# OxygenLost/dddmr_navigation

Measured on AMD Instinct MI355X. Metric: scored trajectories/sec (N_traj x N_steps), higher is better.
Workload: dtype f32; 1 GPU; C3: 16384 trajectories x 80 steps vs 500000-point cloud, 80-pose prune plan, shipped critic stack; scene_layout=r02, trajectories_per_gpu=16384, steps_per_trajectory=80, parallelism=single, contexts_per_gpu=1

## Files before the change

dddmr_navigation_amd/_capi.py:

```python
from __future__ import annotations

import ctypes as C
import os

MAX_CRITICS = 8
NAME_LEN = 64
ABI_VERSION = 2

OK = 0
ERR_BAD_ARG = -1
ERR_NO_DEVICE = -2
ERR_HIP = -3
ERR_UNKNOWN_THEORY = -4
ERR_CAPACITY = -5
ERR_STATE = -6
OPINION_PASS = 0
OPINION_PATH_BLOCKED_WAIT = 1

TF_FAIL = 0
PRUNE_PLAN_FAIL = 1
ALL_TRAJECTORIES_FAIL = 2
PERCEPTION_MALFUNCTION = 3
TRAJECTORY_FOUND = 4
PATH_BLOCKED_WAIT = 5
# ... 291 lines not shown
_get = (_int, [_ctx, _vp, _sz, _pn])
_get_of = (_int, [_ctx, _i32, _vp, _sz, _pn])
_fixed = (_int, [_ctx, _vp, _sz])
_plain = (_int, [_ctx])

_TABLE = {
    "create": (_int, [_P(RolloutConfig), _P(_ctx)]),
    "destroy": (None, [_ctx]),
    "set_cloud": (_int, [_ctx] + _cloud),
    "set_scan": (_int, [_ctx] + _cloud + [_pd, _pd, _dbl, _dbl, _pu]),
    "set_stitcher": (_int, [_ctx, _i32]),
    "get_cloud": _get,
    "set_prune_plan": _fixed,
    "samples": (_int, [_ctx, _str, _P(TickInput), _vp, _sz, _pn]),
    "tick": (_int, [_ctx, _str, _P(TickInput), _P(RolloutResult)]),
    "tick_begin": (_int, [_ctx, _str, _P(TickInput)]),
    "tick_end": (_int, [_ctx, _P(RolloutResult)]),
    "resolve": (_int, [_ctx, _i64, _P(RolloutResult)]),
    "winner_words": (None, [_P(RolloutResult), _pi64]),
    "resolve_words": (_int, [_ctx, _pi64, _i32, _P(RolloutResult)]),
    "get_debug": (_int, [_ctx, _P(RolloutDebug)]),
    "heading_rows": _plain,
    "fused_walk": _plain,
    "get_best_poses": _get,
    "get_best_cuboids": _get,
    "get_pose_arrays": _get_of,
    "path_blocked": (_int, [_ctx, _vp, _sz, _dbl, _pd, _P(_i32), _vp]),
    "pack_key": (_i64, [_dbl, _u32]),
    "key_index": (_i32, [_i64]),
    "comm_unique_id": (_int, [_vp]),
    "comm_init": (_int, [_ctx, _vp, _i32, _i32]),
    "comm_destroy": _plain,
    "comm_ranks": (_int, [_ctx, _P(_i32)]),
    "device_count": (_int, [_P(_i32)]),
    "comm_loopback": _plain,
    "comm_loopback_set_peer": (_int, [_ctx, _i32, _pi64]),
    "marking_create": (_int, [_ctx, _P(MarkingConfig)] + _cloud + _cloud),
    "marking_update": (_int, [_ctx, _pd, _pd, _P(MarkingStats)]),
    "marking_reset": _plain,
    "marking_get_voxels": _get,
    "marking_get_points": (_int, [_ctx, _vp, _vp, _sz, _pn]),
    "marking_get_dgraph": _fixed,
    "marking_get_lethal": _fixed,
    "marking_route_counts": (_int, [_ctx, _pu, _pu, _pu]),
    "set_scan_source": (_int, [_ctx, _i32] + _cloud + [_pd, _pd, _dbl, _dbl, _pu, _pu]),
    "set_stitcher_source": (_int, [_ctx, _i32, _i32]),
# ... 86 lines not shown
```

dddmr_navigation_amd/csrc/rollout_engine.hip:

```cpp
#include <hip/hip_runtime.h>
#include <dlfcn.h>
#include <rccl/rccl.h>

#include <algorithm>
#include <atomic>
#include <cmath>
#include <cstdarg>
#include <chrono>
#include <cstdio>
#include <cstdlib>
#include <cstring>
#include <memory>
#include <mutex>
#include <string>
#include <vector>

#include "rollout_kernels.hip.h"
#include "tick_plan.hip.h"
#include "perception_kernels.hip.h"
#include "depth_feed.hip.h"
#include "depth_image.hip.h"
#include "depth_clear.hip.h"
#include "lidar_sweep.hip.h"
#include "lidar_features.hip.h"
// ... 96 lines not shown
  bool comm_loopback = false;
  int64_t* slots_dev = nullptr;
  int64_t* slots_red = nullptr;
  DevResult* local_result_dev = nullptr;

  ModuleSlot<MarkingState> marking;
  ModuleSlot<DepthMarkState> dmark;
  ModuleSlot<DepthLayerState> dlayer;
  ModuleSlot<StackState> stack;
  ModuleSlot<MclState> mcl;

  std::mutex tick_mu;
  std::mutex err_mu;
  std::string last_error;

  DevTick last{};
  bool have_last = false;
  Window last_window;
  int timing = 1;
  int timing_every = 1;
  int spin = 1;
  int last_heading_rows = -1;
  int last_fused_walk = -1;
  uint32_t seq = 0;
  DevResult last_result{};
  float last_score_ms = 0.f, last_device_ms = 0.f;
  struct Pending {
    bool active = false;
    TickPlan plan;
    bool timed = false, timed_all = false;
    Window window;
  } pend;
};

namespace {

class CloudPin {
 public:
  enum Mode { kFront, kOfPendingTick, kAdopted };
  explicit CloudPin(dddmr_rollout_ctx* c, Mode mode = kFront) : c_(c), owns_(mode != kOfPendingTick) {
    if (mode == kAdopted) {
      idx_ = c_->busy;
      return;
    }
    std::lock_guard<std::mutex> lk(c_->cloud_mu);
    if (mode == kFront) {
// ... 64 lines not shown
}
#define TICK_IDLE(ctx, what)                        \
  std::lock_guard<std::mutex> tk((ctx)->tick_mu);   \
  if ((ctx)->pend.active) return refuse_pending(ctx, what)

const dddmr_theory_config* find_theory(const dddmr_rollout_ctx* ctx, const char* name) {
  for (const auto& t : ctx->theories)
    if (std::strncmp(t.name, name, DDDMR_NAME_LEN) == 0) return &t;
  return nullptr;
}

void read_env(dddmr_rollout_ctx* ctx) {
  TickKnobs& kn = ctx->knobs;
  if (const char* e = std::getenv("DDDMR_CELL")) {
    const float v = (float)std::atof(e);
    if (v > 0.01f && v < 10.f) { kn.cell_size = v; kn.cell_forced = true; }
  }
  if (const char* e = std::getenv("DDDMR_TILE")) kn.tile_override = std::atoi(e);
  if (const char* e = std::getenv("DDDMR_RT")) kn.rt_override = std::atoi(e);
  if (const char* e = std::getenv("DDDMR_THREADS")) kn.threads_override = std::atoi(e) == 512 ? 512 : 256;
  if (const char* e = std::getenv("DDDMR_TAIL_ROUND")) kn.tail_round = std::atoi(e) != 0;
  if (const char* e = std::getenv("DDDMR_HEADING_ROWS")) kn.heading_rows = std::atoi(e) != 0;
  if (const char* e = std::getenv("DDDMR_FUSE_WALK")) kn.fuse_walk = std::atoi(e) != 0;
  if (const char* e = std::getenv("DDDMR_FINAL")) kn.final_mode = std::atoi(e) ? 1 : 0;
  if (const char* e = std::getenv("DDDMR_PROBE")) kn.probe_mode = std::atoi(e) ? 1 : 0;
  if (const char* e = std::getenv("DDDMR_TIMING")) ctx->timing = std::atoi(e);
  if (const char* e = std::getenv("DDDMR_TIMING_EVERY")) ctx->timing_every = std::max(1, std::atoi(e));
  if (const char* e = std::getenv("DDDMR_SPIN")) ctx->spin = std::atoi(e);
  const struct { const char* name; bool* on; } given[] = {
      {"DDDMR_NO_ASSIGN", &kn.no_assign}, {"DDDMR_NO_BOXFAST", &kn.no_boxfast}, {"DDDMR_NO_TAB", &kn.no_tab},
      {"DDDMR_GNZ_ONE", &kn.gnz_one},     {"DDDMR_POISON", &ctx->poison},       {"DDDMR_HOST_PROF", &ctx->host_prof},
      {"DDDMR_DEBUG_GRID", &ctx->debug_grid}};
  for (const auto& g : given) *g.on = std::getenv(g.name) != nullptr;
  if (const char* e = std::getenv("DDDMR_CEIL_BLOCKS")) ctx->ceil_blocks = std::max(1, std::atoi(e));
}

}

#include "rollout_comm.hip.h"

extern "C" {

const char* dddmr_rollout_version(void) { return "dddmr-rollout-mi355x 0.1 (gfx950)"; }

size_t dddmr_rollout_sizeof(int which) {
  switch (which) {
// ... 123 lines not shown
    HIPCHK(ctx, dev_alloc(mem, &ctx->steps, N));
    HIPCHK(ctx, dev_alloc(mem, &ctx->samples_out, N));
    HIPCHK(ctx, dev_alloc(mem, &ctx->best_key, (size_t)kSlotBase + (size_t)kSlotWords * N));
    HIPCHK(ctx, dev_alloc(mem, &ctx->overflow, 1));
    HIPCHK(ctx, dev_alloc(mem, &ctx->traj_load, N));
    HIPCHK(ctx, hipMemset(ctx->traj_load, 0, N * sizeof(uint32_t)));
    HIPCHK(ctx, dev_alloc(mem, &ctx->assign, N));
    HIPCHK(ctx, dev_alloc(mem, &ctx->tickets, 2));
    HIPCHK(ctx, hipMemset(ctx->tickets, 0, 2 * sizeof(uint32_t)));
    HIPCHK(ctx, dev_alloc(mem, &ctx->poses_dev, (size_t)cfg->max_steps * 7));
    HIPCHK(ctx, dev_alloc(mem, &ctx->blocked_plan, (size_t)kBlockedMaxPlan));
    HIPCHK(ctx, dev_alloc(mem, &ctx->blocked_flags, (size_t)kBlockedMaxPlan / 32));
    for (int i = 0; i < kCloudBufs; ++i) HIPCHK(ctx, host_alloc(ctx->host, &ctx->cloud_stage[i], P * sizeof(float4)));
    const size_t small = std::max<size_t>({3 * kMaxAxis * sizeof(float), N * sizeof(float4),
                                           plan_cap * sizeof(float4)});
    HIPCHK(ctx, host_alloc(ctx->host, &ctx->small_stage, small));
    if (host_mapped_alloc(ctx->host, &ctx->result_host, &ctx->result_dev, sizeof(DevResult)) != 0)
      return fail(ctx, DDDMR_ERR_HIP, "result record allocation failed");
    const int rc = perception_alloc(ctx->feed, P);
    if (rc != 0) return fail(ctx, DDDMR_ERR_HIP, "perception scratch allocation failed");
    {
      const void* big_lds_kernels[] = {
          reinterpret_cast<const void*>(k_rollout), reinterpret_cast<const void*>(k_bin_count),
          reinterpret_cast<const void*>(k_score<256, false, false>), reinterpret_cast<const void*>(k_score<256, false, true>),
          reinterpret_cast<const void*>(k_score<256, true, false>),  reinterpret_cast<const void*>(k_score<256, true, true>),
          reinterpret_cast<const void*>(k_score<512, false, false>), reinterpret_cast<const void*>(k_score<512, false, true>),
          reinterpret_cast<const void*>(k_score<512, true, false>),  reinterpret_cast<const void*>(k_score<512, true, true>)};
      for (const void* f : big_lds_kernels) HIPCHK(ctx, hipFuncSetAttribute(f, hipFuncAttributeMaxDynamicSharedMemorySize, kScoreLdsMax));
    }
    HIPCHK(ctx, hipDeviceSynchronize());
    return DDDMR_OK;
  };
  const int rc = init();
  if (rc != DDDMR_OK) {
    fprintf(stderr, "dddmr_rollout_create: %s\n", ctx->last_error.c_str());
    dddmr_rollout_destroy(ctx);
    return rc;
  }
  *out = ctx;
  return DDDMR_OK;
}

static void publish_cloud(dddmr_rollout_ctx* ctx, int idx, uint32_t n, const SourceLayout& layout) {
  std::lock_guard<std::mutex> lk(ctx->cloud_mu);
  ctx->cloud_n[idx] = n;
  ctx->cloud_layout[idx] = layout;
  ctx->front = idx;
  ctx->wait_pending[idx] = true;
}

// ... 198 lines not shown
      ctx->st_cap = cap;
      if (!ctx->traj_info) HIPCHK(ctx, dev_alloc(ctx->mem, &ctx->traj_info, (size_t)ctx->cfg.max_trajectories));
    }
  }
  HIPCHK(ctx, pin.wait_on(ctx->stream));

  const auto prof_t1 = std::chrono::steady_clock::now();
  if (ctx->poison && k.n_local > 0) {
    HIPCHK(ctx, hipMemsetAsync(ctx->costs, 0xFF, (size_t)k.n_local * sizeof(double), ctx->stream));
    HIPCHK(ctx, hipMemsetAsync(ctx->steps, 0xFF, (size_t)k.n_local * sizeof(int32_t), ctx->stream));
    HIPCHK(ctx, hipMemsetAsync(ctx->samples_out, 0xFF, (size_t)k.n_local * sizeof(float4), ctx->stream));
    HIPCHK(ctx, hipMemsetAsync(ctx->partial, 0xFF, (size_t)k.n_local * sizeof(TrajPartial), ctx->stream));
    HIPCHK(ctx, hipMemsetAsync(ctx->st_pp, 0xFF, (size_t)k.n_local * sizeof(double2), ctx->stream));
  }
  k.seq = ++ctx->seq;
  if (k.seq == 0) k.seq = ctx->seq = 1;
  const bool timed = ctx->timing >= 1 && (ctx->seq % (uint32_t)ctx->timing_every) == 0;
  const bool timed_all = timed && ctx->timing >= 2;
  if (timed_all) HIPCHK(ctx, hipEventRecord(ctx->ev0, ctx->stream));
  ctx->feedback.load_theory = theory_id;
  ctx->feedback.load_nlocal = k.n_local;
  ctx->last_heading_rows = p.heading_rows;
  ctx->last_fused_walk = k.n_local > 0 ? p.fused_walk : 0;
  drain.armed = true;
  if (k.n_points > 0) {
    hipLaunchKernelGGL(k_bin_count, dim3(p.cnt_blocks + p.roll_blocks + (k.use_assign ? k.assign_groups : 0)), dim3(kBinThreads),
                       p.roll_launch_lds, ctx->stream, k, pin.dev(), ctx->cell_count, ctx->cell_start, ctx->pt_slot, ctx->tickets,
                       ctx->best_key, ctx->overflow, ctx->axes_dev, ctx->samples_dev, ctx->traj_info, ctx->st_sc,
                       ctx->st_xy, ctx->st_pp, ctx->traj_load, ctx->assign, p.heading_rows);
    hipLaunchKernelGGL(k_bin_scatter, dim3(p.bin_blocks), dim3(256), 0, ctx->stream, k, pin.dev(),
                       ctx->pt_slot, ctx->cell_start, ctx->sorted, ctx->row_tab);
  } else {
    hipLaunchKernelGGL(k_bin_reset, dim3(1), dim3(256), 0, ctx->stream, k, ctx->cell_count, ctx->cell_start,
                       ctx->best_key, ctx->overflow);
    if (p.roll_blocks > 0)
      hipLaunchKernelGGL(k_rollout, dim3(p.roll_blocks), dim3(256), p.roll_launch_lds, ctx->stream, k, ctx->axes_dev,
                         ctx->samples_dev, ctx->traj_info, ctx->st_sc, ctx->st_xy, ctx->st_pp, p.heading_rows);
    if (k.use_assign)
      hipLaunchKernelGGL(k_assign, dim3(k.assign_groups), dim3(kBinThreads), 0, ctx->stream, k, ctx->traj_load, ctx->assign);
  }
  if (timed) HIPCHK(ctx, hipEventRecord(ctx->evs0, ctx->stream));
  DevResult* score_result = exchange ? ctx->local_result_dev : ctx->result_dev;
  int64_t* score_words = exchange ? ctx->slots_dev + 2 * p.rank : nullptr;
  if (k.n_local > 0) {
    const int wgs = k.n_tiles;
    const size_t lds = p.score_lds;
#define DDDMR_LAUNCH_SCORE(T, L)                                                                                   \
  do { if (k.probe) DDDMR_LAUNCH_SCORE_P(T, L, true); else DDDMR_LAUNCH_SCORE_P(T, L, false); } while (0)
#define DDDMR_LAUNCH_SCORE_P(T, L, P)                                                                              \
  hipLaunchKernelGGL((k_score<T, L, P>), dim3(wgs), dim3(T), lds, ctx->stream, k, ctx->traj_info, ctx->st_sc,     \
                     ctx->st_xy, ctx->plan_dev, ctx->cell_start, ctx->sorted, ctx->costs, ctx->steps,             \
                     ctx->samples_out, ctx->best_key, ctx->overflow, ctx->tickets + 1, score_result, ctx->assign, \
                     ctx->traj_load, score_words, ctx->row_tab, ctx->plan_pairs_dev, ctx->partial, p.fused_walk,  \
                     ctx->st_pp)
    if (p.thr == 512) { if (p.lean) DDDMR_LAUNCH_SCORE(512, true); else DDDMR_LAUNCH_SCORE(512, false); }
    else              { if (p.lean) DDDMR_LAUNCH_SCORE(256, true); else DDDMR_LAUNCH_SCORE(256, false); }
#undef DDDMR_LAUNCH_SCORE
#undef DDDMR_LAUNCH_SCORE_P
  } else {
    hipLaunchKernelGGL(k_empty_result, dim3(1), dim3(64), 0, ctx->stream, k, ctx->cell_start, score_result, score_words);
  }
  if (timed) HIPCHK(ctx, hipEventRecord(ctx->evs1, ctx->stream));
  if (k.n_local > 0 && k.final_kernel)
    hipLaunchKernelGGL(k_finalize, dim3((k.n_local + kFinalThreads - 1) / kFinalThreads), dim3(kFinalThreads), 0, ctx->stream, k,
                       ctx->traj_info, ctx->partial, ctx->costs, ctx->steps, ctx->samples_out, ctx->traj_load, ctx->best_key,
                       ctx->cell_start, ctx->overflow, ctx->tickets + 1, score_result, score_words);
  if (exchange) {
    if (ctx->comm) {
      const int nrc = rccl().all_reduce(ctx->slots_dev, ctx->slots_red, (size_t)2 * ctx->comm_ranks, ncclInt64, ncclMin,
                                        ctx->comm, ctx->stream);
      if (nrc != ncclSuccess) return fail(ctx, DDDMR_ERR_HIP, "ncclAllReduce failed: %s", rccl().error_string((ncclResult_t)nrc));
    } else {
      HIPCHK(ctx, hipMemcpyAsync(ctx->slots_red, ctx->slots_dev, (size_t)2 * ctx->comm_ranks * sizeof(int64_t),
                                 hipMemcpyDeviceToDevice, ctx->stream));
    }
    hipLaunchKernelGGL(k_resolve, dim3(1), dim3(64), 0, ctx->stream, k, ctx->slots_red, ctx->comm_ranks,
                       ctx->local_result_dev, ctx->axes_dev, ctx->samples_dev, ctx->result_dev);
  }
  if (timed_all) HIPCHK(ctx, hipEventRecord(ctx->ev1, ctx->stream));
  HIPCHK(ctx, hipGetLastError());
  if (ctx->host_prof) {
// ... 159 lines not shown
  if (!th) return fail(ctx, DDDMR_ERR_UNKNOWN_THEORY, "unknown theory '%s'", theory_name);
  Window w;
  make_window(*th, *in, w);
  const size_t n = w.count();
  *n_samples = n;
  if (!samples_out) return DDDMR_OK;
  if (capacity < n) return fail(ctx, DDDMR_ERR_CAPACITY, "samples: capacity %zu < %zu", capacity, n);
  for (size_t i = 0; i < n; ++i) sample_of(w, (int)i, samples_out + 3 * i, samples_out + 3 * i + 1, samples_out + 3 * i + 2);
  return DDDMR_OK;
}

int dddmr_rollout_heading_rows(dddmr_rollout_ctx* ctx) {
  if (!ctx) return -1;
  std::lock_guard<std::mutex> tk(ctx->tick_mu);
  return ctx->last_heading_rows;
}

int dddmr_rollout_fused_walk(dddmr_rollout_ctx* ctx) {
  if (!ctx) return -1;
  std::lock_guard<std::mutex> tk(ctx->tick_mu);
  return ctx->last_fused_walk;
}

int dddmr_rollout_get_debug(dddmr_rollout_ctx* ctx, dddmr_rollout_debug* dbg) {
  if (!ctx || !dbg) return DDDMR_ERR_BAD_ARG;
  std::lock_guard<std::mutex> tk(ctx->tick_mu);
  if (!ctx->have_last) return fail(ctx, DDDMR_ERR_STATE, "get_debug before any tick");
  if (ctx->pend.active) return refuse_pending(ctx, "get_debug");
  HIPCHK(ctx, hipSetDevice(ctx->device));
  HIPCHK(ctx, hipStreamSynchronize(ctx->stream));
  const size_t n = (size_t)ctx->last.n_local;
  if (n == 0) return DDDMR_OK;
  if (dbg->costs) HIPCHK(ctx, hipMemcpy(dbg->costs, ctx->costs, n * sizeof(double), hipMemcpyDeviceToHost));
  if (dbg->steps) HIPCHK(ctx, hipMemcpy(dbg->steps, ctx->steps, n * sizeof(int32_t), hipMemcpyDeviceToHost));
  if (dbg->samples) {
    std::vector<float4> tmp(n);
    HIPCHK(ctx, hipMemcpy(tmp.data(), ctx->samples_out, n * sizeof(float4), hipMemcpyDeviceToHost));
    for (size_t i = 0; i < n; ++i) {
      dbg->samples[3 * i + 0] = tmp[i].x;
      dbg->samples[3 * i + 1] = tmp[i].y;
      dbg->samples[3 * i + 2] = tmp[i].z;
    }
  }
  return DDDMR_OK;
}

// ... 104 lines not shown
```

dddmr_navigation_amd/csrc/rollout_kernels.hip.h:

```cpp
#pragma once
#include <hip/hip_runtime.h>
#include <limits.h>
#include <stdint.h>

#include "../../include/dddmr_rollout.h"

#pragma clang fp contract(off)

namespace dddmr {

#ifndef DDDMR_PSPLIT_MAX
#define DDDMR_PSPLIT_MAX 4
#endif
#ifndef DDDMR_SCORE_WPE
#define DDDMR_SCORE_WPE 2
#endif
#ifndef DDDMR_SCORE_WPE_256
#define DDDMR_SCORE_WPE_256 5
#endif
#ifdef DDDMR_HANDOFF_ACQREL
#define DDDMR_HANDOFF_ORDER __ATOMIC_ACQ_REL
#else
#define DDDMR_HANDOFF_ORDER __ATOMIC_RELAXED
#endif
// ... 620 lines not shown
  for (int idx = tid; idx < nt * S1; idx += kThreads) {
    const int j = bj, s = bs;
    bj += stride_j;
    bs += stride_s;
    if (bs >= S1) { bs -= S1; ++bj; }
    if (s < steps_s[j]) {
      const float* slot = reinterpret_cast<const float*>(inc + idx);
      st_xy[(size_t)li_s[j] * k.max_steps + s] = make_float2(slot[0], slot[2]);
    }
  }
  if (tid < nt) {
    const int ns = steps_s[tid];
    double2 pp = make_double2(0.0, 0.0);
    if (ns > 0) {
      const float* slot = reinterpret_cast<const float*>(inc + (size_t)tid * S1 + (ns - 1));
      const double2 cs = shared ? hrow[(int)lc_s[tid] * S1 + ns] : inc[(size_t)tid * S1 + ns];
      pp = pure_pursuit_last_pose(k, make_float2(slot[0], slot[2]), cs);
    }
    st_pp[li_s[tid]] = pp;
  }
  DDDMR_RSTAMP(3);
}

__device__ __forceinline__ int tile_round_base(const DevTick& k, int r) {
  return r < k.r0 ? r * k.nb_tiles : k.r0 * k.nb_tiles + (r - k.r0) * k.n_tiles;
}
__device__ __forceinline__ int tile_slot(const DevTick& k, int b, int j) {
  return tile_round_base(k, b < k.nb_tiles ? j : j + k.r0) + b;
}
constexpr int kAssignPer = 4;
template <int kThreads>
__device__ __forceinline__ void assign_block(const DevTick& k, const int grp, const uint32_t* __restrict__ load,
                                             uint32_t* __restrict__ assign) {
  __shared__ uint32_t hist[kLoadClasses];
  __shared__ uint32_t wsum[kThreads / 64];
  __shared__ uint32_t mx_s, mn_s;
  static_assert(kLoadClasses == kThreads, "one class per lane in the scan");
  const int tid = threadIdx.x;
  const int G = k.assign_groups;
  const int n = k.n_local, tl = k.n_tiles / G, tlb = k.nb_tiles / G;
  const int ng = (n - grp + G - 1) / G;
  auto group_slot = [&](int r) {
    const int early = k.r0 * tlb;
    int start, width, round;
    if (r < early) { round = r / tlb; start = round * tlb; width = tlb; }
    else { round = k.r0 + (r - early) / tl; start = early + (round - k.r0) * tl; width = tl; }
    const int pos = r - start;
    const int bl = ((round & 1) && start + width <= ng) ? width - 1 - pos : pos;
    return grp + G * (start + bl);
  };
  DDDMR_RSTAMP(0);
  hist[tid] = 0;
  if (tid == 0) { mx_s = 1; mn_s = 0xFFFFFFFFu; }
  uint32_t v[kAssignPer];
  uint32_t mx = 1, mn = 0xFFFFFFFFu;
#pragma unroll
  for (int e = 0; e < kAssignPer; ++e) {
    const int m = tid + e * kThreads;
    v[e] = m < ng ? load[grp + G * m] : 0u;
    if (m < ng) { mx = max(mx, v[e]); mn = min(mn, v[e]); }
  }
#pragma unroll
  for (int o = 32; o > 0; o >>= 1) {
    mx = max(mx, (uint32_t)__shfl_xor((int)mx, o, 64));
    mn = min(mn, (uint32_t)__shfl_xor((int)mn, o, 64));
  }
  __syncthreads();
  if ((tid & 63) == 0) { atomicMax(&mx_s, mx); atomicMin(&mn_s, mn); }
  __syncthreads();
  if (mx_s <= mn_s) {
#pragma unroll
    for (int e = 0; e < kAssignPer; ++e) {
      const int m = tid + e * kThreads;
// ... 2 lines not shown
    return;
  }
  const float scale = (float)(kLoadClasses - 1) / (float)mx_s;
#pragma unroll
  for (int e = 0; e < kAssignPer; ++e) {
    const int m = tid + e * kThreads;
    if (m < ng) atomicAdd(&hist[kLoadClasses - 1 - min(kLoadClasses - 1, (int)((float)v[e] * scale))], 1u);
  }
  __syncthreads();
  const uint32_t cnt = hist[tid];
  const uint32_t inc = wave_incl_scan_u32(cnt);
  if ((tid & 63) == 63) wsum[tid >> 6] = inc;
  __syncthreads();
  uint32_t base = inc - cnt;
  for (int w = 0; w < (tid >> 6); ++w) base += wsum[w];
  hist[tid] = base;
  __syncthreads();
#pragma unroll
  for (int e = 0; e < kAssignPer; ++e) {
    const int m = tid + e * kThreads;
    if (m < ng) {
      const int c = kLoadClasses - 1 - min(kLoadClasses - 1, (int)((float)v[e] * scale));
      const int r = (int)atomicAdd(&hist[c], 1u);
      assign[group_slot(r)] = (uint32_t)(grp + G * m);
    }
  }
  DDDMR_RSTAMP(3);
}

__global__ __launch_bounds__(kBinThreads) void k_assign(DevTick k, const uint32_t* __restrict__ load,
                                                        uint32_t* __restrict__ assign) {
  assign_block<kBinThreads>(k, (int)blockIdx.x, load, assign);
}

__global__ __launch_bounds__(256) void k_rollout(DevTick k, const float* __restrict__ axes,
                                                 const float4* __restrict__ samples,
                                                 TrajInfo* __restrict__ info, double2* __restrict__ st_sc,
                                                 float2* __restrict__ st_xy, double2* __restrict__ st_pp,
                                                 const int heading_rows) {
  extern __shared__ __attribute__((aligned(16))) unsigned char dyn_lds[];
  rollout_block<256>(k, (int)blockIdx.x, axes, samples, info, st_sc, st_xy, st_pp, dyn_lds, heading_rows != 0);
}

__global__ __launch_bounds__(kBinThreads, 8) void k_bin_count(DevTick k, const float4* __restrict__ cloud,
                                                   uint32_t* __restrict__ cell_count,
                                                   uint32_t* __restrict__ cell_start,
                                                   uint2* __restrict__ pt_slot, uint32_t* __restrict__ ticket,
                                                   int64_t* __restrict__ best_key,
                                                   uint32_t* __restrict__ overflow, const float* __restrict__ axes,
                                                   const float4* __restrict__ samples, TrajInfo* __restrict__ info,
                                                   double2* __restrict__ st_sc, float2* __restrict__ st_xy,
                                                   double2* __restrict__ st_pp, const uint32_t* __restrict__ load,
                                                   uint32_t* __restrict__ assign, const int heading_rows) {
  extern __shared__ __attribute__((aligned(16))) unsigned char dyn_lds[];
  const int n_assign = k.use_assign ? k.assign_groups : 0;
  if ((int)blockIdx.x < n_assign) {
    assign_block<kBinThreads>(k, (int)blockIdx.x, load, assign);
    return;
  }
  if ((int)blockIdx.x < n_assign + k.roll_blocks) {
    rollout_block<kBinThreads>(k, (int)blockIdx.x - n_assign, axes, samples, info, st_sc, st_xy, st_pp, dyn_lds, heading_rows != 0);
    return;
  }
  const int bin_block = (int)blockIdx.x - n_assign - k.roll_blocks;
  __shared__ uint32_t wave_sum[16];
  __shared__ uint32_t carry_s;
  __shared__ uint32_t is_last;
  const int stride = k.bin_blocks * blockDim.x;
  DDDMR_RSTAMP(0);
  for (int base = bin_block * blockDim.x + threadIdx.x; base < k.n_points; base += stride * kBinPer) {
    float4 p[kBinPer];
    uint2 slot[kBinPer];
#pragma unroll
    for (int m = 0; m < kBinPer; ++m) {
      const int i = base + m * stride;
      p[m] = i < k.n_points ? cloud[i] : make_float4(0.f, 0.f, 0.f, 0.f);
    }
#pragma unroll
    for (int m = 0; m < kBinPer; ++m) {
      const int i = base + m * stride;
// ... 318 lines not shown
    *result = r;
    if (words_out) {
      words_out[0] = any ? (int64_t)bc : kKeyNone;
      words_out[1] = any ? -(int64_t)r.index : kKeyNone;
    } else {
      __threadfence_system();
      __hip_atomic_store(&result->seq, k.seq, __ATOMIC_RELEASE, __HIP_MEMORY_SCOPE_SYSTEM);
    }
    if (kStamps) DDDMR_STAMP_RAW(18);
  }
}

__device__ __forceinline__ double stick_sum_wave(const float* dr, const int ns, const int lane) {
  double acc = 0.0;
  for (int s2 = lane; s2 < ns; s2 += 64) acc += (double)dr[s2];
  acc += dpp_row_shl<8>(acc);
  acc += dpp_row_shl<4>(acc);
  acc += dpp_row_shl<2>(acc);
  acc += dpp_row_shl<1>(acc);
  const double r1 = __shfl(acc, 16, 64), r2 = __shfl(acc, 32, 64), r3 = __shfl(acc, 48, 64);
  return (acc + r1) + (r2 + r3);
}

template <int kScoreThreads, bool kLean, bool kProbe>
__global__ __launch_bounds__(kScoreThreads, kScoreThreads >= 512 ? DDDMR_SCORE_WPE : DDDMR_SCORE_WPE_256) void k_score(
    DevTick k, const TrajInfo* __restrict__ info, const double2* __restrict__ st_sc, const float2* __restrict__ st_xy,
    const float4* __restrict__ plan_xyz, const uint32_t* __restrict__ cell_start,
    const Pt3* __restrict__ sorted, double* __restrict__ costs, int32_t* __restrict__ steps_out,
    float4* __restrict__ samples_out, int64_t* __restrict__ best_key, uint32_t* __restrict__ overflow,
    uint32_t* __restrict__ ticket, DevResult* __restrict__ result, const uint32_t* __restrict__ assign,
    uint32_t* __restrict__ traj_load, int64_t* __restrict__ words_out, const uint32_t* __restrict__ row_tab,
    const float* __restrict__ plan_pairs, TrajPartial* __restrict__ partial, const int fused_walk,
    const double2* __restrict__ st_pp) {
  extern __shared__ __attribute__((aligned(16))) unsigned char lds_raw[];
  const int tile = k.tile;
  const int S1 = k.max_steps + 1;
  const int Qcap = tile * k.max_steps;
  constexpr bool kCanFuse = kLean && kScoreThreads == 512;
  const bool fused = kCanFuse && fused_walk != 0 && Qcap <= kScoreThreads && k.m > 0 && k.want_collision != 0 && k.n_points >= 5;
  const bool need_box = k.want_collision != 0, need_mm = !kLean && k.want_minmax != 0;
  const bool rec_pose = !kLean && k.rec_pose != 0;
  const bool box_fast = kLean || k.box_fast != 0;
  const int rec_words = rec_words_of(rec_pose, need_mm);
  const int mm_ofs = kRecBase + (rec_pose ? 3 : 0);
  size_t ofs = 0;
  TrajHead* head = reinterpret_cast<TrajHead*>(lds_raw);
  ofs += sizeof(TrajHead) * (size_t)tile;
  ofs = (ofs + 15) & ~(size_t)15;
  float4* plan = reinterpret_cast<float4*>(lds_raw + ofs);
  ofs += 16 * (size_t)(k.m > 0 ? k.m : 1);
  float4* ppos = reinterpret_cast<float4*>(lds_raw + ofs);
  ofs += 16 * (size_t)Qcap;
  float* dist = reinterpret_cast<float*>(lds_raw + ofs);
  ofs += 4 * (size_t)tile * S1;
  float* rec = reinterpret_cast<float*>(lds_raw + ofs);
  ofs += 4 * (size_t)rec_words * Qcap;
// ... 481 lines not shown
        const int i1 = min(k.m, i + per);
        for (; i + 4 <= i1; i += 4) {
          const float4 p0 = plan[i], p1 = plan[i + 1], p2 = plan[i + 2], p3 = plan[i + 3];
          const f2 da = l2_simple2(f2{p0.x, p1.x}, f2{p0.y, p1.y}, f2{p0.z, p1.z}, px, py, pz);
          const f2 db = l2_simple2(f2{p2.x, p3.x}, f2{p2.y, p3.y}, f2{p2.z, p3.z}, px, py, pz);
          best = fminf(fminf(best, fminf(da.x, da.y)), fminf(db.x, db.y));
        }
        for (; i < i1; ++i) {
          const float4 pp = plan[i];
          best = fminf(best, l2_simple(pp.x, pp.y, pp.z, px, py, pz));
        }
      }
      if (G > 1) best = fminf(best, dpp_row_shl<1>(best));
      if (G > 2) best = fminf(best, dpp_row_shl<2>(best));
      if (G > 4) best = fminf(best, dpp_row_shl<4>(best));
      if (G > 8) best = fminf(best, dpp_row_shl<8>(best));
      if (valid && g == 0) dist[(size_t)j * S1 + s] = sqrtf(best);
    }
  }
  __syncthreads();
  }
  DDDMR_STAMP(8);

  if (k.final_kernel) {
    for (int j = wid; j < nt; j += kScoreThreads / 64) {
      const int ns = head[j].steps;
      const double sum = stick_sum_wave(dist + (size_t)j * S1, ns, lane);
      if (lane == 0) {
        const bool hb = head[j].hit_box != 0, hm = head[j].hit_mm != 0;
        const bool dead = cloud_ok && ((need_box && hb) || (need_mm && hm));
        TrajPartial* pr = partial + head[j].li;
        pr->stick_sum = dead ? 0.0 : sum;
        pr->pp_dist = head[j].pp_dist;
        pr->pp_yaw = head[j].pp_yaw;
        pr->dist_last = (ns > 0 && !dead) ? dist[(size_t)j * S1 + ns - 1] : 0.f;
        pr->flags = partial_flags(head[j].walked, hb, hm);
      }
    }
    DDDMR_STAMP(10);
    DDDMR_STAMP(11);
    DDDMR_STAMP(7);
    return;
  }
  for (int j = wid; j < nt; j += kScoreThreads / 64) {
    const double sum = stick_sum_wave(dist + (size_t)j * S1, head[j].steps, lane);
    if (lane == 0) head[j].stick_sum = sum;
  }
  __syncthreads();
  DDDMR_STAMP(10);

  int64_t cbits = kKeyNone;
  int my_gi = -1;
  if (tid < nt) {
    const TrajHead h = head[tid];
    const int li = head[tid].li;
    const int gi = k.begin + li;
    my_gi = gi;
    const bool hb = h.hit_box != 0, hm = h.hit_mm != 0;
    const bool dead = cloud_ok && ((need_box && hb) || (need_mm && hm));
    double cost = DDDMR_COST_NOT_GENERATED;
    if (h.steps > 0) {
      const float dist_last = dead ? 0.f : dist[(size_t)tid * S1 + h.steps - 1];
      StackArgs sa;
      stack_args_load(k, sa);
      asm volatile("" : "+s"(sa.kind), "+s"(sa.w), "+s"(sa.tw), "+s"(sa.ow));
      cost = score_stack(k, sa, h.w, h.steps, hb, hm, h.stick_sum, h.pp_dist, h.pp_yaw, dist_last, &cbits);
    }
    costs[li] = cost;
    samples_out[li] = make_float4(h.vx, h.vy, h.w, 0.f);
    steps_out[li] = h.steps;
    traj_load[li] = traj_load_of(k.m, h.walked, h.steps, (need_box && hb) || (need_mm && hm));
  }
  DDDMR_STAMP(11);
  unsigned long long* slots = reinterpret_cast<unsigned long long*>(best_key) + kSlotBase;
  if (tid < 64) {
    long long cc = (long long)cbits;
    int gi_w = my_gi;
    {
      long long oc; int oi; bool take;
      oc = dpp_row_shl<8>(cc); oi = dpp_row_shl<8>(gi_w); take = oc < cc || (oc == cc && oi > gi_w); cc = take ? oc : cc; gi_w = take ? oi : gi_w;
      oc = dpp_row_shl<4>(cc); oi = dpp_row_shl<4>(gi_w); take = oc < cc || (oc == cc && oi > gi_w); cc = take ? oc : cc; gi_w = take ? oi : gi_w;
      oc = dpp_row_shl<2>(cc); oi = dpp_row_shl<2>(gi_w); take = oc < cc || (oc == cc && oi > gi_w); cc = take ? oc : cc; gi_w = take ? oi : gi_w;
      oc = dpp_row_shl<1>(cc); oi = dpp_row_shl<1>(gi_w); take = oc < cc || (oc == cc && oi > gi_w); cc = take ? oc : cc; gi_w = take ? oi : gi_w;
    }
    const int win_gi = __builtin_amdgcn_readfirstlane(gi_w);
    const bool gen = tid < nt && head[tid].steps > 0;
    const bool coll = gen && cloud_ok && ((need_box && head[tid].hit_box) || (need_mm && head[tid].hit_mm));
    const unsigned long long cm = __ballot(coll), gm = __ballot(gen);
    const unsigned long long wm = __ballot(tid < nt && my_gi == win_gi);
    if (tid == 0) {
      float vx = 0.f, vy = 0.f, w = 0.f;
      if (cc != (long long)kKeyNone && wm) {
        const int wl = __ffsll((long long)wm) - 1;
        vx = head[wl].vx; vy = head[wl].vy; w = head[wl].w;
// ... 265 lines not shown
```

dddmr_navigation_amd/csrc/tick_plan.hip.h:

```cpp
#pragma once
#include <algorithm>
#include <cmath>
#include <cstring>
#include <string>
#include <vector>

#include "rollout_kernels.hip.h"

using namespace dddmr;

namespace {

constexpr uint32_t kCapCells = 1u << 20;
constexpr int kMaxAxis = 4096;
constexpr int kScoreLdsMax = 150 * 1024;

struct Window {
  std::vector<float> ax, ay, ath;
  bool list_mode = false;
  std::vector<float4> list;
  size_t count() const { return list_mode ? list.size() : ax.size() * ay.size() * ath.size(); }
};

void velocity_samples(double lo, double hi, int n, bool insert_zero, std::vector<float>& out) {
// ... 166 lines not shown
  } else {
    const int nth = (int)w.ath.size(), ny = (int)w.ay.size();
    *vx = w.ax[(idx / nth) / ny];
    *vy = w.ay[(idx / nth) % ny];
    *wz = w.ath[idx % nth];
  }
}

struct TickKnobs {
  float cell_size = 0.25f;
  bool cell_forced = false;
  bool gnz_one = false;
  int tile_override = 0;
  int threads_override = 0;
  int rt_override = 0;
  bool tail_round = false;
  int final_mode = -1;
  int probe_mode = -1;
  bool no_assign = false;
  bool no_boxfast = false;
  bool no_tab = false;
  bool heading_rows = true;
  bool fuse_walk = true;
  int n_cu = 256;
};

struct TickFeedback {
  int load_theory = -1, load_nlocal = -1;
  float collided_share = 1.0f;
};

enum SampleUpload {
  kUploadNone = 0,
  kUploadList,
  kUploadAxesInline,
  kUploadAxesDev
};

struct TickPlan {
  DevTick k{};
  int s_tick = 0;
  int rank = 0;
  int thr = 512;
  size_t score_lds = 0;
  bool lean = false;
  int cnt_blocks = 0;
  int bin_blocks = 0;
  int roll_blocks = 0;
  size_t roll_lds = 0;
  int heading_rows = 0;
  size_t roll_launch_lds = 0;
  int fused_walk = 0;
  SampleUpload upload = kUploadNone;
  uint32_t n_samples = 0, local_begin = 0, n_local = 0;
};

inline float fused_walk_share_max(int pairs) { return 1.0f - 256.0f / (float)pairs; }

size_t plan_score_lds(const DevTick& k, int tile) {
  return score_lds_bytes(tile, k.max_steps, k.m, rec_words_of(k.rec_pose != 0, k.want_minmax != 0), k.tab_entries, k.rows_cap);
}

int plan_tick(const TickKnobs& kn, const TickFeedback& fb, const dddmr_rollout_config& cfg, const dddmr_theory_config& th,
              int theory_id, const dddmr_tick_input& in, const Window& w, uint32_t n_points, uint32_t plan_m,
              const double plan_last[7], bool exchange, TickPlan* p, std::string* err) {
  const size_t N = w.count();
  if (N > cfg.max_trajectories) {
    *err = std::to_string(N) + " samples > max_trajectories " + std::to_string(cfg.max_trajectories);
    return DDDMR_ERR_CAPACITY;
  }
  if (!w.list_mode && (w.ax.size() > (size_t)kMaxAxis || w.ay.size() > (size_t)kMaxAxis || w.ath.size() > (size_t)kMaxAxis)) {
    *err = "sample axis longer than " + std::to_string(kMaxAxis);
    return DDDMR_ERR_CAPACITY;
  }
  const int world = std::max(1, cfg.world_size);
// ... 230 lines not shown
  k.bin_blocks = p->cnt_blocks;
  k.roll_blocks = p->roll_blocks;
  k.n_tiles = k.n_local > 0 ? (k.n_local + tile - 1) / tile : 0;
  k.assign_groups = std::max(1, (k.n_local + kAssignPer * kBinThreads - 1) / (kAssignPer * kBinThreads));
  k.use_assign = (!kn.no_assign && k.n_tiles > 1 && k.n_local <= kAssignMax && same_as_last) ? 1 : 0;
  if (k.use_assign) k.n_tiles = (k.n_tiles + k.assign_groups - 1) / k.assign_groups * k.assign_groups;
  k.nb_tiles = k.n_tiles;
  k.r0 = 0;
  if (!one_round && tile > 1 && kn.tail_round && k.n_local <= kAssignMax) {
    const int G = k.assign_groups;
    const long slots = (long)kn.n_cu * (thr == 512 ? 2 : 4);
    const long whole = (long)k.n_local / (slots * tile);
    const long rem = (long)k.n_local - whole * slots * tile;
    const int t2 = (int)((rem + slots - 1) / slots);
    if (whole >= 1 && rem > 0 && t2 < tile) {
      const int nb = (int)((whole * slots + G - 1) / G * G), ns = (int)((slots + G - 1) / G * G);
      if ((long)nb * tile + (long)ns * t2 >= k.n_local) {
        k.nb_tiles = nb;
        k.n_tiles = nb + ns;
        k.r0 = tile - t2;
      }
    }
  }
  return DDDMR_OK;
}

}
```

dddmr_navigation_amd/local_planner.py:

```python
from __future__ import annotations

import ctypes as C
import enum
from dataclasses import dataclass
from typing import Iterable, Optional

import numpy as np

from . import _capi as K
from . import _marshal as M
from . import configs


class PlannerState(enum.IntEnum):
    TF_FAIL = 0
    PRUNE_PLAN_FAIL = 1
    ALL_TRAJECTORIES_FAIL = 2
    PERCEPTION_MALFUNCTION = 3
    TRAJECTORY_FOUND = 4
    PATH_BLOCKED_WAIT = 5
    PATH_BLOCKED_REPLANNING = 6


@dataclass
class Trajectory:
    xv_: float = 0.0
    yv_: float = 0.0
    thetav_: float = 0.0
    cost_: float = -1.0
    index: int = -1


class RolloutError(RuntimeError):
    def __init__(self, code: int, msg: str):
        super().__init__(f"dddmr_rollout error {code}: {msg}")
        self.code = code


def device_count() -> int:
    n = C.c_int32(0)
    rc = K.load_library().dddmr_rollout_device_count(C.byref(n))
    return int(n.value) if rc == K.OK else 0


class LocalPlanner:

    def __init__(self, theories: Iterable[K.TheoryConfig], device: int = 0, max_points: int = 600_000,
                 max_trajectories: int = 65_536, max_steps: int = 256, max_plan_poses: int = 256,
                 rank: int = 0, world_size: int = 1):
        self._lib = K.load_library()
        self._theories = configs.theory_array(theories)
        cfg = K.RolloutConfig()
        cfg.abi_version = K.ABI_VERSION
        cfg.device = device
        cfg.rank = rank
        cfg.world_size = world_size
        cfg.max_points = max_points
        cfg.max_trajectories = max_trajectories
        cfg.max_steps = max_steps
        cfg.max_plan_poses = max_plan_poses
        cfg.n_theories = len(self._theories)
        cfg.theories = C.cast(self._theories, C.POINTER(K.TheoryConfig))
        self._ctx = C.c_void_p()
        rc = self._lib.dddmr_rollout_create(C.byref(cfg), C.byref(self._ctx))
        if rc != K.OK:
# ... 372 lines not shown
```

include/dddmr_rollout.h:

```cpp
#ifndef DDDMR_ROLLOUT_H_
#define DDDMR_ROLLOUT_H_

#include <stddef.h>
#include <stdint.h>

#ifdef __cplusplus
extern "C" {
#endif

#define DDDMR_ROLLOUT_ABI_VERSION 2
#define DDDMR_MAX_CRITICS 8
#define DDDMR_NAME_LEN 64
#define DDDMR_COMM_ID_BYTES 128

typedef enum {
  DDDMR_OK = 0,
  DDDMR_ERR_BAD_ARG = -1,
  DDDMR_ERR_NO_DEVICE = -2,
  DDDMR_ERR_HIP = -3,
  DDDMR_ERR_UNKNOWN_THEORY = -4,
  DDDMR_ERR_CAPACITY = -5,
  DDDMR_ERR_STATE = -6
} dddmr_status;

// ... 311 lines not shown
                             const dddmr_tick_input* in);
int dddmr_rollout_tick_end(dddmr_rollout_ctx* ctx, dddmr_rollout_result* out);

int dddmr_rollout_resolve(dddmr_rollout_ctx* ctx, int64_t reduced_key,
                          dddmr_rollout_result* inout);
void dddmr_rollout_winner_words(const dddmr_rollout_result* r, int64_t words[2]);
int dddmr_rollout_resolve_words(dddmr_rollout_ctx* ctx, const int64_t* words, int32_t n_ranks,
                                dddmr_rollout_result* inout);

int dddmr_rollout_comm_unique_id(uint8_t id_out[DDDMR_COMM_ID_BYTES]);
int dddmr_rollout_comm_init(dddmr_rollout_ctx* ctx, const uint8_t id[DDDMR_COMM_ID_BYTES],
                            int32_t rank, int32_t n_ranks);
int dddmr_rollout_comm_destroy(dddmr_rollout_ctx* ctx);
int dddmr_rollout_device_count(int32_t* n_out);
int dddmr_rollout_comm_ranks(dddmr_rollout_ctx* ctx, int32_t* n_ranks_out);
int dddmr_rollout_comm_loopback(dddmr_rollout_ctx* ctx);
int dddmr_rollout_comm_loopback_set_peer(dddmr_rollout_ctx* ctx, int32_t peer_rank, const int64_t words[2]);

int dddmr_rollout_get_debug(dddmr_rollout_ctx* ctx, dddmr_rollout_debug* dbg);

int dddmr_rollout_heading_rows(dddmr_rollout_ctx* ctx);

int dddmr_rollout_fused_walk(dddmr_rollout_ctx* ctx);

int dddmr_rollout_get_pose_arrays(dddmr_rollout_ctx* ctx, int32_t which, double* poses_out,
                                  size_t capacity, size_t* n_poses);

int dddmr_rollout_get_best_poses(dddmr_rollout_ctx* ctx, double* poses_out,
                                 size_t capacity, size_t* n_poses);

int dddmr_rollout_get_best_cuboids(dddmr_rollout_ctx* ctx, float* vertices_out, size_t capacity_poses,
                                   size_t* n_poses);

int64_t dddmr_rollout_pack_key(double cost, uint32_t global_index);
int32_t dddmr_rollout_key_index(int64_t key);

typedef struct {
  double xy_resolution, height_resolution;
  double marking_height, perception_window_size;
  double vertical_FOV_top, vertical_FOV_bottom;
  double scan_effective_positive_start, scan_effective_positive_end;
  double scan_effective_negative_start, scan_effective_negative_end;
  double euclidean_cluster_extraction_tolerance;
  int32_t euclidean_cluster_extraction_min_cluster_size;
  int32_t reserved;
  double segmentation_ignore_ratio;
// ... 135 lines not shown
```

Measured before the change: 127.3 million trajectories/s.

## Deal trajectories to score tiles in sorted load order using per-trajectory collision-item counts

```diff
diff --git a/dddmr_navigation_amd/_capi.py b/dddmr_navigation_amd/_capi.py
--- a/dddmr_navigation_amd/_capi.py
+++ b/dddmr_navigation_amd/_capi.py
@@ -337,6 +337,8 @@
     "get_debug": (_int, [_ctx, _P(RolloutDebug)]),
     "heading_rows": _plain,
     "fused_walk": _plain,
+    "deal": _plain,
+    "get_deal": (_int, [_ctx, _vp, _vp, _sz, _pn, _P(_i32)]),
     "get_best_poses": _get,
     "get_best_cuboids": _get,
     "get_pose_arrays": _get_of,
diff --git a/dddmr_navigation_amd/csrc/rollout_engine.hip b/dddmr_navigation_amd/csrc/rollout_engine.hip
--- a/dddmr_navigation_amd/csrc/rollout_engine.hip
+++ b/dddmr_navigation_amd/csrc/rollout_engine.hip
@@ -142,6 +142,8 @@
   int spin = 1;
   int last_heading_rows = -1;
   int last_fused_walk = -1;
+  int last_deal = -1;
+  int last_assigned = 0;
   uint32_t seq = 0;
   DevResult last_result{};
   float last_score_ms = 0.f, last_device_ms = 0.f;
@@ -252,6 +254,7 @@
   if (const char* e = std::getenv("DDDMR_TAIL_ROUND")) kn.tail_round = std::atoi(e) != 0;
   if (const char* e = std::getenv("DDDMR_HEADING_ROWS")) kn.heading_rows = std::atoi(e) != 0;
   if (const char* e = std::getenv("DDDMR_FUSE_WALK")) kn.fuse_walk = std::atoi(e) != 0;
+  if (const char* e = std::getenv("DDDMR_DEAL")) kn.deal_mode = std::min(std::max(std::atoi(e), -1), 2);
   if (const char* e = std::getenv("DDDMR_FINAL")) kn.final_mode = std::atoi(e) ? 1 : 0;
   if (const char* e = std::getenv("DDDMR_PROBE")) kn.probe_mode = std::atoi(e) ? 1 : 0;
   if (const char* e = std::getenv("DDDMR_TIMING")) ctx->timing = std::atoi(e);
@@ -421,10 +424,11 @@
     {
       const void* big_lds_kernels[] = {
           reinterpret_cast<const void*>(k_rollout), reinterpret_cast<const void*>(k_bin_count),
-          reinterpret_cast<const void*>(k_score<256, false, false>), reinterpret_cast<const void*>(k_score<256, false, true>),
-          reinterpret_cast<const void*>(k_score<256, true, false>),  reinterpret_cast<const void*>(k_score<256, true, true>),
-          reinterpret_cast<const void*>(k_score<512, false, false>), reinterpret_cast<const void*>(k_score<512, false, true>),
-          reinterpret_cast<const void*>(k_score<512, true, false>),  reinterpret_cast<const void*>(k_score<512, true, true>)};
+#define DDDMR_SCORE_KERNELS(T, L) \
+  reinterpret_cast<const void*>(k_score<T, L, false, false>), reinterpret_cast<const void*>(k_score<T, L, true, false>), \
+  reinterpret_cast<const void*>(k_score<T, L, false, true>), reinterpret_cast<const void*>(k_score<T, L, true, true>)
+          DDDMR_SCORE_KERNELS(256, false), DDDMR_SCORE_KERNELS(256, true), DDDMR_SCORE_KERNELS(512, false), DDDMR_SCORE_KERNELS(512, true)};
+#undef DDDMR_SCORE_KERNELS
       for (const void* f : big_lds_kernels) HIPCHK(ctx, hipFuncSetAttribute(f, hipFuncAttributeMaxDynamicSharedMemorySize, kScoreLdsMax));
     }
     HIPCHK(ctx, hipDeviceSynchronize());
@@ -669,12 +673,14 @@
   ctx->feedback.load_nlocal = k.n_local;
   ctx->last_heading_rows = p.heading_rows;
   ctx->last_fused_walk = k.n_local > 0 ? p.fused_walk : 0;
+  ctx->last_deal = p.deal;
+  ctx->last_assigned = k.use_assign;
   drain.armed = true;
   if (k.n_points > 0) {
     hipLaunchKernelGGL(k_bin_count, dim3(p.cnt_blocks + p.roll_blocks + (k.use_assign ? k.assign_groups : 0)), dim3(kBinThreads),
                        p.roll_launch_lds, ctx->stream, k, pin.dev(), ctx->cell_count, ctx->cell_start, ctx->pt_slot, ctx->tickets,
                        ctx->best_key, ctx->overflow, ctx->axes_dev, ctx->samples_dev, ctx->traj_info, ctx->st_sc,
-                       ctx->st_xy, ctx->st_pp, ctx->traj_load, ctx->assign, p.heading_rows);
+                       ctx->st_xy, ctx->st_pp, ctx->traj_load, ctx->assign, p.heading_rows, p.deal, p.deal_head);
     hipLaunchKernelGGL(k_bin_scatter, dim3(p.bin_blocks), dim3(256), 0, ctx->stream, k, pin.dev(),
                        ctx->pt_slot, ctx->cell_start, ctx->sorted, ctx->row_tab);
   } else {
@@ -684,7 +690,8 @@
       hipLaunchKernelGGL(k_rollout, dim3(p.roll_blocks), dim3(256), p.roll_launch_lds, ctx->stream, k, ctx->axes_dev,
                          ctx->samples_dev, ctx->traj_info, ctx->st_sc, ctx->st_xy, ctx->st_pp, p.heading_rows);
     if (k.use_assign)
-      hipLaunchKernelGGL(k_assign, dim3(k.assign_groups), dim3(kBinThreads), 0, ctx->stream, k, ctx->traj_load, ctx->assign);
+      hipLaunchKernelGGL(k_assign, dim3(k.assign_groups), dim3(kBinThreads), 0, ctx->stream, k, ctx->traj_load, ctx->assign, p.deal,
+                         p.deal_head);
   }
   if (timed) HIPCHK(ctx, hipEventRecord(ctx->evs0, ctx->stream));
   DevResult* score_result = exchange ? ctx->local_result_dev : ctx->result_dev;
@@ -695,15 +702,18 @@
 #define DDDMR_LAUNCH_SCORE(T, L)                                                                                   \
   do { if (k.probe) DDDMR_LAUNCH_SCORE_P(T, L, true); else DDDMR_LAUNCH_SCORE_P(T, L, false); } while (0)
 #define DDDMR_LAUNCH_SCORE_P(T, L, P)                                                                              \
-  hipLaunchKernelGGL((k_score<T, L, P>), dim3(wgs), dim3(T), lds, ctx->stream, k, ctx->traj_info, ctx->st_sc,     \
+  do { if (p.deal != kDealSnake) DDDMR_LAUNCH_SCORE_K(T, L, P, true); else DDDMR_LAUNCH_SCORE_K(T, L, P, false); } while (0)
+#define DDDMR_LAUNCH_SCORE_K(T, L, P, I)                                                                           \
+  hipLaunchKernelGGL((k_score<T, L, P, I>), dim3(wgs), dim3(T), lds, ctx->stream, k, ctx->traj_info, ctx->st_sc,     \
                      ctx->st_xy, ctx->plan_dev, ctx->cell_start, ctx->sorted, ctx->costs, ctx->steps,             \
                      ctx->samples_out, ctx->best_key, ctx->overflow, ctx->tickets + 1, score_result, ctx->assign, \
                      ctx->traj_load, score_words, ctx->row_tab, ctx->plan_pairs_dev, ctx->partial, p.fused_walk,  \
-                     ctx->st_pp)
+                     ctx->st_pp, p.deal)
     if (p.thr == 512) { if (p.lean) DDDMR_LAUNCH_SCORE(512, true); else DDDMR_LAUNCH_SCORE(512, false); }
     else              { if (p.lean) DDDMR_LAUNCH_SCORE(256, true); else DDDMR_LAUNCH_SCORE(256, false); }
 #undef DDDMR_LAUNCH_SCORE
 #undef DDDMR_LAUNCH_SCORE_P
+#undef DDDMR_LAUNCH_SCORE_K
   } else {
     hipLaunchKernelGGL(k_empty_result, dim3(1), dim3(64), 0, ctx->stream, k, ctx->cell_start, score_result, score_words);
   }
@@ -909,6 +919,36 @@
   return ctx->last_fused_walk;
 }
 
+int dddmr_rollout_deal(dddmr_rollout_ctx* ctx) {
+  if (!ctx) return -1;
+  std::lock_guard<std::mutex> tk(ctx->tick_mu);
+  return ctx->last_deal;
+}
+
+int dddmr_rollout_get_deal(dddmr_rollout_ctx* ctx, uint32_t* assign_out, uint32_t* load_out, size_t capacity, size_t* n_local,
+                           int32_t* assigned) {
+  if (!ctx || !n_local) return DDDMR_ERR_BAD_ARG;
+  std::lock_guard<std::mutex> tk(ctx->tick_mu);
+  if (!ctx->have_last) return fail(ctx, DDDMR_ERR_STATE, "get_deal before any tick");
+  if (ctx->pend.active) return refuse_pending(ctx, "get_deal");
+  const size_t n = (size_t)ctx->last.n_local;
+  *n_local = n;
+  if (assigned) *assigned = ctx->last_assigned;
+  if ((!assign_out && !load_out) || n == 0) return DDDMR_OK;
+  if (capacity < n) return fail(ctx, DDDMR_ERR_CAPACITY, "get_deal: capacity %zu < %zu", capacity, n);
+  HIPCHK(ctx, hipSetDevice(ctx->device));
+  HIPCHK(ctx, hipStreamSynchronize(ctx->stream));
+  if (assign_out) {
+    if (ctx->last_assigned) {
+      HIPCHK(ctx, hipMemcpy(assign_out, ctx->assign, n * sizeof(uint32_t), hipMemcpyDeviceToHost));
+    } else {
+      for (size_t i = 0; i < n; ++i) assign_out[i] = (uint32_t)i;
+    }
+  }
+  if (load_out) HIPCHK(ctx, hipMemcpy(load_out, ctx->traj_load, n * sizeof(uint32_t), hipMemcpyDeviceToHost));
+  return DDDMR_OK;
+}
+
 int dddmr_rollout_get_debug(dddmr_rollout_ctx* ctx, dddmr_rollout_debug* dbg) {
   if (!ctx || !dbg) return DDDMR_ERR_BAD_ARG;
   std::lock_guard<std::mutex> tk(ctx->tick_mu);
diff --git a/dddmr_navigation_amd/csrc/rollout_kernels.hip.h b/dddmr_navigation_amd/csrc/rollout_kernels.hip.h
--- a/dddmr_navigation_amd/csrc/rollout_kernels.hip.h
+++ b/dddmr_navigation_amd/csrc/rollout_kernels.hip.h
@@ -666,25 +666,18 @@
   DDDMR_RSTAMP(3);
 }
 
-__device__ __forceinline__ int tile_round_base(const DevTick& k, int r) {
+__host__ __device__ __forceinline__ int tile_round_base(const DevTick& k, int r) {
   return r < k.r0 ? r * k.nb_tiles : k.r0 * k.nb_tiles + (r - k.r0) * k.n_tiles;
 }
-__device__ __forceinline__ int tile_slot(const DevTick& k, int b, int j) {
+__host__ __device__ __forceinline__ int tile_slot(const DevTick& k, int b, int j) {
   return tile_round_base(k, b < k.nb_tiles ? j : j + k.r0) + b;
 }
-constexpr int kAssignPer = 4;
-template <int kThreads>
-__device__ __forceinline__ void assign_block(const DevTick& k, const int grp, const uint32_t* __restrict__ load,
-                                             uint32_t* __restrict__ assign) {
-  __shared__ uint32_t hist[kLoadClasses];
-  __shared__ uint32_t wsum[kThreads / 64];
-  __shared__ uint32_t mx_s, mn_s;
-  static_assert(kLoadClasses == kThreads, "one class per lane in the scan");
-  const int tid = threadIdx.x;
+enum { kDealSnake = 0, kDealSorted = 1, kDealLightTail = 2 };
+__host__ __device__ inline int deal_slot(const DevTick& k, const int grp, const int r, const int deal, const int head) {
   const int G = k.assign_groups;
-  const int n = k.n_local, tl = k.n_tiles / G, tlb = k.nb_tiles / G;
-  const int ng = (n - grp + G - 1) / G;
-  auto group_slot = [&](int r) {
+  const int tl = k.n_tiles / G, tlb = k.nb_tiles / G;
+  const int ng = (k.n_local - grp + G - 1) / G;
+  if (deal == kDealSnake || k.r0 > 0) {
     const int early = k.r0 * tlb;
     int start, width, round;
     if (r < early) { round = r / tlb; start = round * tlb; width = tlb; }
@@ -692,7 +685,36 @@
     const int pos = r - start;
     const int bl = ((round & 1) && start + width <= ng) ? width - 1 - pos : pos;
     return grp + G * (start + bl);
-  };
+  }
+  const int q = ng / tl, rem = ng - q * tl;
+  if (deal == kDealSorted) {
+    const int big = rem * (q + 1);
+    int bl, j;
+    if (r < big) { bl = r / (q + 1); j = r - bl * (q + 1); }
+    else { const int d = (r - big) / q; bl = rem + d; j = r - big - d * q; }
+    return grp + G * (j * tl + bl);
+  }
+  const int hd = head < 0 ? 0 : (head > tl ? tl : head);
+  const int n_head = q * hd + (rem < hd ? rem : hd);
+  const int lo = r < n_head ? 0 : hd, width = r < n_head ? hd : tl - hd;
+  const int rr = r < n_head ? r : r - n_head;
+  int round, pos;
+  if (rr < q * width) { round = rr / width; pos = rr - round * width; if (round & 1) pos = width - 1 - pos; }
+  else { round = q; pos = rr - q * width; }
+  return grp + G * (round * tl + lo + pos);
+}
+
+constexpr int kAssignPer = 4;
+template <int kThreads>
+__device__ __forceinline__ void assign_block(const DevTick& k, const int grp, const uint32_t* __restrict__ load,
+                                             uint32_t* __restrict__ assign, const int deal, const int deal_head) {
+  __shared__ uint32_t hist[kLoadClasses];
+  __shared__ uint32_t wsum[kThreads / 64];
+  __shared__ uint32_t mx_s, mn_s;
+  static_assert(kLoadClasses == kThreads, "one class per lane in the scan");
+  const int tid = threadIdx.x;
+  const int G = k.assign_groups;
+  const int ng = (k.n_local - grp + G - 1) / G;
   DDDMR_RSTAMP(0);
   hist[tid] = 0;
   if (tid == 0) { mx_s = 1; mn_s = 0xFFFFFFFFu; }
@@ -741,15 +763,15 @@
     if (m < ng) {
       const int c = kLoadClasses - 1 - min(kLoadClasses - 1, (int)((float)v[e] * scale));
       const int r = (int)atomicAdd(&hist[c], 1u);
-      assign[group_slot(r)] = (uint32_t)(grp + G * m);
+      assign[deal_slot(k, grp, r, deal, deal_head)] = (uint32_t)(grp + G * m);
     }
   }
   DDDMR_RSTAMP(3);
 }
 
 __global__ __launch_bounds__(kBinThreads) void k_assign(DevTick k, const uint32_t* __restrict__ load,
-                                                        uint32_t* __restrict__ assign) {
-  assign_block<kBinThreads>(k, (int)blockIdx.x, load, assign);
+                                                        uint32_t* __restrict__ assign, const int deal, const int deal_head) {
+  assign_block<kBinThreads>(k, (int)blockIdx.x, load, assign, deal, deal_head);
 }
 
 __global__ __launch_bounds__(256) void k_rollout(DevTick k, const float* __restrict__ axes,
@@ -770,11 +792,12 @@
                                                    const float4* __restrict__ samples, TrajInfo* __restrict__ info,
                                                    double2* __restrict__ st_sc, float2* __restrict__ st_xy,
                                                    double2* __restrict__ st_pp, const uint32_t* __restrict__ load,
-                                                   uint32_t* __restrict__ assign, const int heading_rows) {
+                                                   uint32_t* __restrict__ assign, const int heading_rows,
+                                                   const int deal, const int deal_head) {
   extern __shared__ __attribute__((aligned(16))) unsigned char dyn_lds[];
   const int n_assign = k.use_assign ? k.assign_groups : 0;
   if ((int)blockIdx.x < n_assign) {
-    assign_block<kBinThreads>(k, (int)blockIdx.x, load, assign);
+    assign_block<kBinThreads>(k, (int)blockIdx.x, load, assign, deal, deal_head);
     return;
   }
   if ((int)blockIdx.x < n_assign + k.roll_blocks) {
@@ -1139,7 +1162,7 @@
   return (acc + r1) + (r2 + r3);
 }
 
-template <int kScoreThreads, bool kLean, bool kProbe>
+template <int kScoreThreads, bool kLean, bool kProbe, bool kItemsKey>
 __global__ __launch_bounds__(kScoreThreads, kScoreThreads >= 512 ? DDDMR_SCORE_WPE : DDDMR_SCORE_WPE_256) void k_score(
     DevTick k, const TrajInfo* __restrict__ info, const double2* __restrict__ st_sc, const float2* __restrict__ st_xy,
     const float4* __restrict__ plan_xyz, const uint32_t* __restrict__ cell_start,
@@ -1148,7 +1171,7 @@
     uint32_t* __restrict__ ticket, DevResult* __restrict__ result, const uint32_t* __restrict__ assign,
     uint32_t* __restrict__ traj_load, int64_t* __restrict__ words_out, const uint32_t* __restrict__ row_tab,
     const float* __restrict__ plan_pairs, TrajPartial* __restrict__ partial, const int fused_walk,
-    const double2* __restrict__ st_pp) {
+    const double2* __restrict__ st_pp, const int deal) {
   extern __shared__ __attribute__((aligned(16))) unsigned char lds_raw[];
   const int tile = k.tile;
   const int S1 = k.max_steps + 1;
@@ -1676,6 +1699,12 @@
   }
   DDDMR_STAMP(8);
 
+  const bool key_items = kItemsKey && deal != kDealSnake;
+  const bool have_items = do_coll && total_pairs > 0;
+  auto work_of = [&](const int j) {
+    if (!key_items) return head[j].walked;
+    return have_items ? (int)min(t_item0[j + 1] - t_item0[j], 0x3FFFFFFFu) : 0;
+  };
   if (k.final_kernel) {
     for (int j = wid; j < nt; j += kScoreThreads / 64) {
       const int ns = head[j].steps;
@@ -1688,7 +1717,7 @@
         pr->pp_dist = head[j].pp_dist;
         pr->pp_yaw = head[j].pp_yaw;
         pr->dist_last = (ns > 0 && !dead) ? dist[(size_t)j * S1 + ns - 1] : 0.f;
-        pr->flags = partial_flags(head[j].walked, hb, hm);
+        pr->flags = partial_flags(work_of(j), hb, hm);
       }
     }
     DDDMR_STAMP(10);
@@ -1723,7 +1752,7 @@
     costs[li] = cost;
     samples_out[li] = make_float4(h.vx, h.vy, h.w, 0.f);
     steps_out[li] = h.steps;
-    traj_load[li] = traj_load_of(k.m, h.walked, h.steps, (need_box && hb) || (need_mm && hm));
+    traj_load[li] = traj_load_of(k.m, work_of(tid), h.steps, (need_box && hb) || (need_mm && hm));
   }
   DDDMR_STAMP(11);
   unsigned long long* slots = reinterpret_cast<unsigned long long*>(best_key) + kSlotBase;
diff --git a/dddmr_navigation_amd/csrc/tick_plan.hip.h b/dddmr_navigation_amd/csrc/tick_plan.hip.h
--- a/dddmr_navigation_amd/csrc/tick_plan.hip.h
+++ b/dddmr_navigation_amd/csrc/tick_plan.hip.h
@@ -212,6 +212,7 @@
   bool no_tab = false;
   bool heading_rows = true;
   bool fuse_walk = true;
+  int deal_mode = -1;
   int n_cu = 256;
 };
 
@@ -241,6 +242,8 @@
   int heading_rows = 0;
   size_t roll_launch_lds = 0;
   int fused_walk = 0;
+  int deal = 0;
+  int deal_head = 0;
   SampleUpload upload = kUploadNone;
   uint32_t n_samples = 0, local_begin = 0, n_local = 0;
 };
@@ -517,6 +520,14 @@
       }
     }
   }
+  {
+    const bool layout_ok = k.use_assign && k.r0 == 0;
+    const long slots = (long)kn.n_cu * (thr == 512 ? 2 : 4);
+    p->deal = kDealSnake;
+    if (kn.deal_mode < 0) { if (layout_ok && !one_round && tile > 1) p->deal = kDealSorted; }
+    else if (kn.deal_mode > 0 && layout_ok) p->deal = kn.deal_mode == kDealLightTail ? kDealLightTail : kDealSorted;
+    p->deal_head = (p->deal == kDealLightTail) ? (int)(((long)k.n_tiles / slots) * slots / k.assign_groups) : 0;
+  }
   return DDDMR_OK;
 }
 
diff --git a/dddmr_navigation_amd/local_planner.py b/dddmr_navigation_amd/local_planner.py
--- a/dddmr_navigation_amd/local_planner.py
+++ b/dddmr_navigation_amd/local_planner.py
@@ -41,6 +41,19 @@
     n = C.c_int32(0)
     rc = K.load_library().dddmr_rollout_device_count(C.byref(n))
     return int(n.value) if rc == K.OK else 0
+
+
+def deal(lp: "LocalPlanner") -> int:
+    return int(lp._rc("deal"))
+
+
+def deal_arrays(lp: "LocalPlanner"):
+    n, used = C.c_size_t(0), C.c_int32(0)
+    lp._call("get_deal", None, None, 0, C.byref(n), C.byref(used))
+    assign = np.zeros(max(n.value, 1), dtype=np.uint32)
+    load = np.zeros(max(n.value, 1), dtype=np.uint32)
+    lp._call("get_deal", M.ptr(assign), M.ptr(load), assign.size, C.byref(n), C.byref(used))
+    return assign[:n.value], load[:n.value], bool(used.value)
 
 
 class LocalPlanner:
diff --git a/include/dddmr_rollout.h b/include/dddmr_rollout.h
--- a/include/dddmr_rollout.h
+++ b/include/dddmr_rollout.h
@@ -357,6 +357,11 @@
 int dddmr_rollout_heading_rows(dddmr_rollout_ctx* ctx);
 
 int dddmr_rollout_fused_walk(dddmr_rollout_ctx* ctx);
+
+int dddmr_rollout_deal(dddmr_rollout_ctx* ctx);
+
+int dddmr_rollout_get_deal(dddmr_rollout_ctx* ctx, uint32_t* assign_out, uint32_t* load_out, size_t capacity,
+                           size_t* n_local, int32_t* assigned);
 
 int dddmr_rollout_get_pose_arrays(dddmr_rollout_ctx* ctx, int32_t which, double* poses_out,
                                   size_t capacity, size_t* n_poses);
```

Result: faster. 144.5 million trajectories/s, median of 6 (+13.5%).
